# nz0001na/MorphGANformer

Measured on AMD Instinct MI355X. Metric: latent-projection iters/sec @1024^2, k=17 latents, higher is better.
Workload: dtype f32; 1 GPU; configs[1]: single 1024x1024 face per GPU, Wing+LPIPS(squeeze)+MSE literal-mode projection step, noise_mode=random, seeded synthetic weights/targets/landmarks; k=17, z_dim=32, targets_per_gpu=1, parallelism=pair-sharded x1, graph_replay=True, loss_generator_overlap=True, steps_per_forward=32

## Files before the change

### morphganformer_amd/build.py

```python
from __future__ import annotations

import glob
import hashlib
import os
import subprocess
import sys

HERE = os.path.dirname(os.path.abspath(__file__))
ROOT = os.path.dirname(HERE)
CSRC = os.path.join(HERE, "csrc")
OBJ = os.path.join(CSRC, "_obj")
LIB = os.path.join(HERE, "libmgf_hip.so")
SOURCES = ["capi.cpp", "bias_act.hip", "upfirdn2d.hip", "conv_taps.hip", "latent_prep.hip", "attention.hip", "losses.hip", "lpips_stem.hip",
           "embed.hip", "backward.hip", "wino.hip", "wino3.hip", "pointwise.hip", "narrow_conv.hip", "warp.hip", "lbp.hip", "mdf.hip",
           "wino_tconv.hip", "depthwise.hip", "noise_opt.hip"]
HEADERS = [os.path.join(CSRC, "mgf_common.h"), os.path.join(ROOT, "include", "mgf.h")]
HIPCC = os.environ.get("HIPCC", "/opt/rocm/bin/hipcc")
FLAGS = ["--offload-arch=gfx950", "-O3", "-fPIC", "-std=c++17", "-ffp-contract=on", "-Wno-unused-result", "-x", "hip"]
LINK_FLAGS = ["--offload-arch=gfx950", "-shared", "-fPIC"]

_compiler_id = None


def compiler_id() -> str:
    global _compiler_id
    if _compiler_id is None:
        _compiler_id = subprocess.run([HIPCC, "--version"], stdout=subprocess.PIPE, stderr=subprocess.STDOUT, check=True).stdout.decode()
    return _compiler_id


def object_key(src_path: str, flags) -> str:
    h = hashlib.sha256()
    h.update(compiler_id().encode())
    h.update("\0".join(flags).encode())
    for p in [src_path] + HEADERS:
        with open(p, "rb") as f:
            h.update(b"\0" + os.path.basename(p).encode() + b"\0" + f.read())
    return h.hexdigest()[:16]


def _compile_all(obj_dir, flags_for, verbose, force, prune=True):
    os.makedirs(obj_dir, exist_ok=True)
    objs, todo = [], []
    for src in SOURCES:
        sp = os.path.join(CSRC, src)
        flags = flags_for(src)
        op = os.path.join(obj_dir, f"{src}.{object_key(sp, flags)}.o")
        objs.append(op)
        if force or not os.path.exists(op):
            todo.append((src, op, [HIPCC] + flags + ["-c", sp, "-o", op + ".tmp"]))
    procs, finished = [], []

    def start(i):
        src, op, cmd = todo[i]
        if verbose:
            print(" ".join(cmd), flush=True)
        procs.append((src, op, subprocess.Popen(cmd, stdout=subprocess.PIPE, stderr=subprocess.STDOUT)))

    for i in range(min(max_jobs(), len(todo))):
        start(i)
    while len(finished) < len(procs):
        src, op, pr = procs[len(finished)]
        finished.append((src, op, pr, pr.communicate()[0]))
        if len(procs) < len(todo):
            start(len(procs))
    failed = False
    for src, op, pr, out in finished:
        if pr.returncode != 0:
# ... 75 lines not shown
```

### morphganformer_amd/csrc/conv_taps.hip

```cpp
#include "mgf_common.h"
#include <vector>

namespace {

typedef float f32x16 __attribute__((ext_vector_type(16)));
typedef __bf16 bf16x8 __attribute__((ext_vector_type(8)));
typedef unsigned u32x4 __attribute__((ext_vector_type(4)));

constexpr int CK = 8;
constexpr int CKB = 16;
template <int WM, int WN> struct Slots {
    static constexpr int XS = WN == 4 ? 20 : (WN == 3 ? 15 : (WN == 1 ? 19 : 11));
    static constexpr int WS = WM == 2 ? 5 : 3;
};

struct Ones { float v[2048]; constexpr Ones() : v() { for (int i = 0; i < 2048; ++i) v[i] = 1.0f; } };
__device__ const Ones g_ones = Ones();

struct ConvParams {
    float* y;
    const float* x;
    const float* wp;
    const float* in_scale;
    const float* out_scale;
    mgf_conv_desc d;
    mgf_epilogue ep;
    int has_ep;
    int tw, rows;
    int tw_magic;
    int tiles_x, tiles_y;
    int fh, fw;
    int dy_min, dx_min;
    int co_tiles;
    int ksplit;
    int chunks_per_split;
    int off32_ok;
    float* partial;
    int fixed_geo;
    const void* wb;
    int xcd_per;
};

__device__ __forceinline__ float epi(const mgf_epilogue& ep, float v, int n, int co, int oy, int ox, int out_h, int out_w,
                                     int64_t yoff) {
    if (ep.noise) {
        float ns = ep.noise_strength ? *ep.noise_strength : 1.0f;
        int nn = ep.noise_n > 1 ? n : 0;
        v += ep.noise[((int64_t)nn * out_h + oy) * out_w + ox] * ns;
    }
    if (ep.bias) v += ep.bias[co];
    if (ep.act == MGF_ACT_LRELU) v = v > 0.f ? v : v * ep.alpha;
    else if (ep.act == MGF_ACT_RELU) v = v > 0.f ? v : 0.f;
    v *= ep.gain;
    if (ep.residual) v += ep.residual[yoff];
    return v;
}

__host__ __device__ constexpr int tconv_group(int t) { return ((t / 3) == 1 ? 2 : 0) + ((t % 3) == 1 ? 1 : 0); }

struct TileCtx { int n, ks, co0, ty0, tx0, c_begin, c_end; };

template <int WM, int WN, int MODE, bool PIPE, int NTP, int AR = 0>
__global__ __launch_bounds__(256, 2) void conv_taps_kernel(ConvParams p) {
    static_assert(AR == 0 || (PIPE && (NTP == 9 || NTP == 10)), "bf16x3: the pipelined 3x3 / transposed-conv instantiations only");
    constexpr bool FX = NTP == 10 || NTP == 11;
    constexpr int FXW = NTP == 10 ? 33 : 65;
    constexpr int NT = FX ? 9 : NTP;
    constexpr int CO_T = 32 * WM, PX = 128 * WN, NG = MODE == 1 ? 4 : 1;
    constexpr int CKK = AR ? CKB : CK;
    extern __shared__ float lds[];
    const mgf_conv_desc& d = p.d;
    const int T = NT > 0 ? NT : d.ntaps;
    int toffs[MGF_MAX_TAPS];
#pragma unroll
    for (int t = 0; t < MGF_MAX_TAPS; ++t) toffs[t] = t < T ? (d.dy[t] - p.dy_min) * p.fw + (d.dx[t] - p.dx_min) : 0;
    const int chs = p.fh * p.fw;
    const int xs_floats = CKK * chs;
    const int xs_region = AR ? xs_floats : (PIPE ? Slots<WM, WN>::XS * 256 : xs_floats);
    const int buf_floats = AR ? xs_region + 144 * CO_T : (PIPE ? xs_region + Slots<WM, WN>::WS * 1024 : xs_floats + T * CK * CO_T);

    const int tid = threadIdx.x, lane = tid & 63, wave = tid >> 6;
    const int l31 = lane & 31, half = lane >> 5;
    const int l31_ = l31, half_ = half;
    const int TW = p.tw;
    const int rows = p.rows;
    const int ptiles = p.tiles_x * p.tiles_y;
    const int total_items = ptiles * p.co_tiles * d.n * p.ksplit;
    const int plane = d.in_h * d.in_w;
    const int wrow4 = CO_T / 4;
    const int wsz4 = T * CK * wrow4;

    auto decode = [&](int w, TileCtx& c) {
        const int cot = w % p.co_tiles;
        int r = w / p.co_tiles;
        const int pt = r % ptiles;
        r /= ptiles;
        c.ks = r % p.ksplit;
        c.n = r / p.ksplit;
        c.co0 = cot * CO_T;
        c.ty0 = (pt / p.tiles_x) * rows;
        c.tx0 = (pt % p.tiles_x) * TW;
        c.c_begin = c.ks * p.chunks_per_split * CKK;
        c.c_end = c.c_begin + p.chunks_per_split * CKK;
        if (c.c_end > d.cin) c.c_end = d.cin;
        c.n = __builtin_amdgcn_readfirstlane(c.n); c.ks = __builtin_amdgcn_readfirstlane(c.ks); c.co0 = __builtin_amdgcn_readfirstlane(c.co0);
        c.ty0 = __builtin_amdgcn_readfirstlane(c.ty0); c.tx0 = __builtin_amdgcn_readfirstlane(c.tx0);
        c.c_begin = __builtin_amdgcn_readfirstlane(c.c_begin); c.c_end = __builtin_amdgcn_readfirstlane(c.c_end);
    };

    int pbase[WN];
#pragma unroll
    for (int g = 0; g < WN; ++g) {
        const int pix = (wave * WN + g) * 32 + l31;
        const int pr = (pix * p.tw_magic) >> 16, pc = pix - pr * TW;
        pbase[g] = pr < rows ? pr * d.istride * p.fw + pc * d.istride : 0;
    }

    f32x16 acc[NG][WM][WN];
    auto zero_acc = [&]() {
#pragma unroll
        for (int q = 0; q < NG; ++q)
#pragma unroll
            for (int m = 0; m < WM; ++m)
#pragma unroll
                for (int g = 0; g < WN; ++g)
#pragma unroll
                    for (int r = 0; r < 16; ++r) acc[q][m][g][r] = 0.f;
    };
    zero_acc();

    constexpr int XS = Slots<WM, WN>::XS, WS = Slots<WM, WN>::WS;
    unsigned xoff[XS];
    int woff[WS], wch[WS];
    __amdgpu_buffer_rsrc_t rx_l = __builtin_amdgcn_make_buffer_rsrc((void*)p.x, 0, 0, 0x00020000);
    const __amdgpu_buffer_rsrc_t rw_l = __builtin_amdgcn_make_buffer_rsrc((void*)p.wp, 0, -1, 0x00020000);
    __amdgpu_buffer_rsrc_t rs_l = __builtin_amdgcn_make_buffer_rsrc((void*)g_ones.v, 0, -1, 0x00020000);
    const int sc_step = p.in_scale ? 4 : 0;
    auto setup_slots = [&](const TileCtx& c) {
        rx_l = __builtin_amdgcn_make_buffer_rsrc((void*)(p.x + (int64_t)c.n * d.cin * plane), 0, (int)(4u * (unsigned)(d.cin * plane)), 0x00020000);
        if (p.in_scale) rs_l = __builtin_amdgcn_make_buffer_rsrc((void*)(p.in_scale + (int64_t)c.n * d.cin), 0, -1, 0x00020000);
#pragma unroll
        for (int j = 0; j < WS; ++j) {
            int i = tid + 256 * j;
            if (i >= wsz4) i = wsz4 - 1;
            const int c4 = i % wrow4;
            const int rest = i / wrow4;
            wch[j] = rest % CK;
            woff[j] = ((rest / CK) * d.cin + wch[j]) * d.cout_pad + c.co0 + c4 * 4;
        }
        const int iy0 = c.ty0 * d.istride + p.dy_min, ix0 = c.tx0 * d.istride + p.dx_min;
        int ch = tid / chs;
        int r = (tid - ch * chs) / p.fw;
        int q = tid - ch * chs - r * p.fw;
        const int dr = 256 / p.fw, dq = 256 - dr * p.fw;
#pragma unroll
        for (int j = 0; j < XS; ++j) {
            const int i = tid + 256 * j;
            const int iy = iy0 + r, ix = ix0 + q;
            xoff[j] = (i < xs_floats && iy >= 0 && iy < d.in_h && ix >= 0 && ix < d.in_w) ? 4u * (unsigned)(ch * plane + iy * d.in_w + ix) : 0xFFFFFFF0u;
            q += dq; r += dr;
            if (q >= p.fw) { q -= p.fw; ++r; }
            if (r >= p.fh) { r -= p.fh; ++ch; }
            if (r >= p.fh) { r -= p.fh; ++ch; }
        }
    };
    float xr[XS];
    float4 wr[WS];
    float wsc[WS];
    auto load_chunk = [&](int c0) {
        const int xso = (int)(4u * (unsigned)(c0 * plane)), wso = (int)(4u * (unsigned)(c0 * d.cout_pad)), sso = c0 * sc_step;
#pragma unroll
        for (int j = 0; j < XS; ++j) xr[j] = __builtin_bit_cast(float, __builtin_amdgcn_raw_buffer_load_b32(rx_l, xoff[j], xso, 0));
#pragma unroll
        for (int j = 0; j < WS; ++j) {
            wr[j] = __builtin_bit_cast(float4, __builtin_amdgcn_raw_buffer_load_b128(rw_l, 4u * (unsigned)woff[j], wso, 0));
            wsc[j] = __builtin_bit_cast(float, __builtin_amdgcn_raw_buffer_load_b32(rs_l, 4u * (unsigned)wch[j], sso, 0));
        }
    };
    auto store_chunk = [&](float* buf) {
#pragma unroll
        for (int j = 0; j < XS; ++j) buf[tid + 256 * j] = xr[j];
        float* Wd = buf + xs_region;
#pragma unroll
        for (int j = 0; j < WS; ++j) {
            float4 v = wr[j];
            v.x *= wsc[j]; v.y *= wsc[j]; v.z *= wsc[j]; v.w *= wsc[j];
            *reinterpret_cast<float4*>(Wd + (tid + 256 * j) * 4) = v;
        }
    };
    constexpr int XI = AR ? 3 : 1;
    constexpr int WSB = AR ? (36 * CO_T + 255) / 256 : 1;
    const int stid = tid;
    const int h_st = __builtin_amdgcn_readfirstlane(stid >> 7), lp = stid & 127;
    unsigned xoffb[XI];
    unsigned woffb[WSB];
    struct StageSet { float x[XI][8]; u32x4 w[WSB]; float4 s[2]; };
    int itr[XI], itq[XI];
    unsigned wbase0[WSB];
    if (AR) {
#pragma unroll
        for (int j = 0; j < XI; ++j) {
            const int px = lp + 128 * j;
            itr[j] = px / p.fw;
            itq[j] = px - itr[j] * p.fw;
            if (px >= chs) itr[j] = 1 << 20;
        }
#pragma unroll
        for (int j = 0; j < WSB; ++j) {
            int i = stid + 256 * j;
            if (i >= 36 * CO_T) i = 36 * CO_T - 1;
            const int cc = i % CO_T, rest = i / CO_T;
            wbase0[j] = 16u * (unsigned)(rest * d.cout_pad + cc);
        }
    }
    const __amdgpu_buffer_rsrc_t rwb_l = __builtin_amdgcn_make_buffer_rsrc((void*)p.wb, 0, -1, 0x00020000);
    auto setup_slots_b = [&](const TileCtx& c) {
        rx_l = __builtin_amdgcn_make_buffer_rsrc((void*)(p.x + (int64_t)c.n * d.cin * plane), 0, (int)(4u * (unsigned)(d.cin * plane)), 0x00020000);
        if (p.in_scale) rs_l = __builtin_amdgcn_make_buffer_rsrc((void*)(p.in_scale + (int64_t)c.n * d.cin), 0, -1, 0x00020000);
        const int iy0 = c.ty0 * d.istride + p.dy_min, ix0 = c.tx0 * d.istride + p.dx_min;
// ... 133 lines not shown
                            acc[q][m][g] = __builtin_amdgcn_mfma_f32_32x32x2f32(fa[t & 1][kk][m], fb[t & 1][kk][g], acc[q][m][g], 0, 0, 0);
            }
        } else {
            for (int t = 0; t < T; ++t) {
                const int toff = (d.dy[t] - p.dy_min) * p.fw + (d.dx[t] - p.dx_min);
#pragma unroll
                for (int kk = 0; kk < CK / 2; ++kk) {
                    float a[WM], b[WN];
#pragma unroll
                    for (int m = 0; m < WM; ++m) a[m] = Ws[(t * CK + 2 * kk) * CO_T + m * 32];
#pragma unroll
                    for (int g = 0; g < WN; ++g) b[g] = Xs[2 * kk * chs + pbase[g] + toff];
#pragma unroll
                    for (int m = 0; m < WM; ++m)
#pragma unroll
                        for (int g = 0; g < WN; ++g)
                            acc[0][m][g] = __builtin_amdgcn_mfma_f32_32x32x2f32(a[m], b[g], acc[0][m][g], 0, 0, 0);
                }
            }
        }
    };

    const bool partial = p.ksplit > 1;
    const bool do_ep = p.has_ep && !partial;
    const float ep_ns = (do_ep && p.ep.noise) ? (p.ep.noise_strength ? *p.ep.noise_strength : 1.0f) : 0.f;
    auto epilogue = [&](const TileCtx& c) {
        const int n = c.n, co0 = c.co0;
        int half = half_, l31 = l31_;
        asm volatile("" : "+v"(half), "+v"(l31));
        float* yn = partial ? p.partial + ((int64_t)c.ks * d.n + n) * ((int64_t)d.cout * d.out_h * d.y_pitch) : p.y + (int64_t)n * d.y_batch;
        const int64_t y_plane = partial ? (int64_t)d.out_h * d.y_pitch : d.y_plane;
        const int choff = partial ? 0 : d.y_choff;
        const float* osc = (p.out_scale && !partial) ? p.out_scale + (int64_t)n * d.out_scale_stride : nullptr;
        if (MODE == 0 && WM == 1 && d.rgb_out) {
            const int rc = d.rgb_channels;
            const float* wr = d.rgb_w + (int64_t)n * rc * d.cout;
            float wv[4][16], osv[16], bv[16];
#pragma unroll
            for (int r = 0; r < 16; ++r) {
                const int co = (r & 3) + 8 * (r >> 2) + 4 * half;
                const bool ok = co < d.cout;
                osv[r] = (osc && ok) ? osc[co] : 1.0f;
                bv[r] = (do_ep && p.ep.bias && ok) ? p.ep.bias[co] : 0.f;
#pragma unroll
                for (int cc = 0; cc < 4; ++cc) wv[cc][r] = (cc < rc && ok) ? wr[cc * d.cout + co] : 0.f;
            }
#pragma unroll
            for (int g = 0; g < WN; ++g) {
                const int pix = (wave * WN + g) * 32 + l31;
                const int pr = (pix * p.tw_magic) >> 16;
                const int ty = c.ty0 + pr, tx = c.tx0 + (pix - pr * TW);
                const int oy = ty * d.ostride + d.oy[0], ox = tx * d.ostride + d.ox[0];
                const bool ovalid = pr < rows && ty < d.tile_h && tx < d.tile_w && oy < d.out_h && ox < d.out_w;
                float nz = 0.f;
                if (do_ep && p.ep.noise && ovalid) nz = p.ep.noise[((int64_t)(p.ep.noise_n > 1 ? n : 0) * d.out_h + oy) * d.out_w + ox] * ep_ns;
                float sum[4] = {0.f, 0.f, 0.f, 0.f};
#pragma unroll
                for (int r = 0; r < 16; ++r) {
                    float v = acc[0][0][g][r] * osv[r];
                    if (do_ep) {
                        v += nz;
                        v += bv[r];
                        if (p.ep.act == MGF_ACT_LRELU) v = v > 0.f ? v : v * p.ep.alpha;
                        else if (p.ep.act == MGF_ACT_RELU) v = v > 0.f ? v : 0.f;
                        v *= p.ep.gain;
                    }
// ... 225 lines not shown
                        mfma_chunk_b(curb);
                        if (more) store_chunk_b(S0, nxtb);
                    } else {
                        if (more) load_chunk(cur.c_begin + (c + 1) * CK);
                        mfma_chunk(curb);
                        if (more) store_chunk(nxtb);
                    }
                    __syncthreads();
                    b ^= 1;
                }
                epilogue(cur);
                zero_acc();
                slot += slot_step;
                if (slot >= slot_end) break;
                decode(wbase + slot, cur);
            }
        }
    } else {
        const int w = p.xcd_per > 0 ? (int)(blockIdx.x & 7) * p.xcd_per + (int)(blockIdx.x >> 3) : (int)blockIdx.x;
        if (w >= total_items || (p.xcd_per > 0 && (int)(blockIdx.x >> 3) >= p.xcd_per)) return;
        TileCtx cur;
        decode(w, cur);
        const int nchunks = (cur.c_end - cur.c_begin + CK - 1) / CK;
        for (int c = 0; c < nchunks; ++c) {
            __syncthreads();
            stage_direct(cur, cur.c_begin + c * CK, lds);
            __syncthreads();
            mfma_chunk(lds);
        }
        epilogue(cur);
    }
}

__global__ __launch_bounds__(256) void splitk_reduce_kernel(ConvParams p) {
    const mgf_conv_desc& d = p.d;
    const int64_t per_n = (int64_t)d.cout * d.out_h * d.out_w;
    const int64_t total = per_n * d.n;
    const int64_t pplane = (int64_t)d.out_h * d.y_pitch;
    const int64_t slice = (int64_t)d.n * d.cout * pplane;
    for (int64_t i = (int64_t)blockIdx.x * 256 + threadIdx.x; i < total; i += (int64_t)gridDim.x * 256) {
        const int ox = (int)(i % d.out_w);
        int64_t r = i / d.out_w;
        const int oy = (int)(r % d.out_h); r /= d.out_h;
        const int co = (int)(r % d.cout);
        const int n = (int)(r / d.cout);
        const int64_t poff = ((int64_t)n * d.cout + co) * pplane + (int64_t)oy * d.y_pitch + ox;
        float v = 0.f;
        const float* pp = p.partial + poff;
        int s = 0;
        for (; s + 8 <= p.ksplit; s += 8) {
            float a[8];
#pragma unroll
            for (int u = 0; u < 8; ++u) a[u] = pp[(int64_t)(s + u) * slice];
#pragma unroll
            for (int u = 0; u < 8; ++u) v += a[u];
        }
        for (; s + 4 <= p.ksplit; s += 4) {
            const float a0 = pp[(int64_t)s * slice], a1 = pp[(int64_t)(s + 1) * slice];
            const float a2 = pp[(int64_t)(s + 2) * slice], a3 = pp[(int64_t)(s + 3) * slice];
            v += a0; v += a1; v += a2; v += a3;
        }
        for (; s < p.ksplit; ++s) v += pp[(int64_t)s * slice];
        if (p.out_scale) v *= p.out_scale[(int64_t)n * d.out_scale_stride + co];
        const int64_t yoff = (int64_t)n * d.y_batch + (int64_t)(d.y_choff + co) * d.y_plane + (int64_t)oy * d.y_pitch + ox;
        if (p.has_ep) v = epi(p.ep, v, n, co, oy, ox, d.out_h, d.out_w, yoff);
        p.y[yoff] = v;
    }
}

struct ProfRec { hipEvent_t e0, e1; int wm, wn, mode, pipe, nt, ksplit; double flops, bytes; const char* name; };
bool g_prof_on = false;
std::vector<ProfRec> g_prof;

struct ProfScope {
    hipStream_t st; bool on;
    ProfScope(hipStream_t s, int wm, int wn, int mode, int pipe, int nt, const ConvParams& p) : st(s), on(g_prof_on) {
        if (!on) return;
        ProfRec r;
        r.name = nullptr;
        r.wm = wm; r.wn = wn; r.mode = mode; r.pipe = pipe; r.nt = nt; r.ksplit = p.ksplit;
        const mgf_conv_desc& d = p.d;
        r.flops = mode == 1 ? 2.0 * 9 * d.cin * (double)d.cout * d.in_h * d.in_w * d.n
                            : 2.0 * d.ntaps * d.cin * (double)d.cout * d.tile_h * d.tile_w * d.n;
        r.bytes = 4.0 * ((double)d.n * d.cin * d.in_h * d.in_w + (double)d.ntaps * d.cin * d.cout +
                         (double)d.n * (d.rgb_out ? d.rgb_channels : d.cout) * d.out_h * d.out_w);
        (void)hipEventCreate(&r.e0); (void)hipEventCreate(&r.e1);
        (void)hipEventRecord(r.e0, st);
        g_prof.push_back(r);
    }
    ~ProfScope() { if (on) (void)hipEventRecord(g_prof.back().e1, st); }
};

template <int MODE>
int launch_conv_bf(const ConvParams& p_in, hipStream_t st) {
    ConvParams p = p_in;
    constexpr int WM = 1, WN = 2, CO_T = 32;
    const int chs = p.fh * p.fw;
    const size_t lds = 2 * ((size_t)16 * chs + (size_t)144 * CO_T) * sizeof(float);
    if (2 * chs > 768 || p.d.cin % CKB != 0 || lds > 80 * 1024) {
        mgf_set_error("conv_taps(bf16x3): footprint %d x %d / %d input channels not supported", p.fh, p.fw, p.d.cin);
        return MGF_EUNSUPPORTED;
    }
    const int64_t items = (int64_t)p.tiles_x * p.tiles_y * p.co_tiles * p.d.n * p.ksplit;
    const int64_t resident = (int64_t)MGF_NUM_CU * 2;
    dim3 grid((unsigned)(items < resident ? items : resident));
    p.xcd_per = 0;
    if (items >= 16) {
        p.xcd_per = (int)((items + 7) / 8);
        if (grid.x % 8 != 0) grid.x = (grid.x + 7) / 8 * 8;
    }
    auto kern1 = conv_taps_kernel<WM, WN, MODE, true, (MODE == 1 ? 10 : 9), 1>;
    static bool attr_set = false;
    if (!attr_set) {
        hipError_t e = hipFuncSetAttribute((const void*)kern1, hipFuncAttributeMaxDynamicSharedMemorySize, 80 * 1024);
        if (e != hipSuccess) { mgf_set_error("conv_taps(bf16x3): cannot raise dynamic LDS: %s", hipGetErrorString(e)); return MGF_ELAUNCH; }
        attr_set = true;
    }
    {
        ProfScope ps(st, WM, WN, MODE, 1, MODE == 1 ? 10 : 9, p);
        if (ps.on) g_prof.back().name = MODE == 1 ? "conv_taps_kernel<1, 2, 1, true, 10, 1>" : "conv_taps_kernel<1, 2, 0, true, 9, 1>";
        hipLaunchKernelGGL(kern1, grid, dim3(256), lds, st, p);
    }
    if (p.ksplit > 1) {
        const int64_t total = (int64_t)p.d.n * p.d.cout * p.d.out_h * p.d.out_w;
        hipLaunchKernelGGL(splitk_reduce_kernel, dim3(mgf_stream_grid(total, 256, 2)), dim3(256), 0, st, p);
    }
    return MGF_OK;
}

template <int WM, int WN, int MODE>
int launch_conv(const ConvParams& p_in, hipStream_t st) {
    ConvParams p = p_in;
    constexpr int CO_T = 32 * WM;
    const size_t buf = ((size_t)CK * p.fh * p.fw + (size_t)p.d.ntaps * CK * CO_T) * sizeof(float);
    const bool pipe = (size_t)CK * p.fh * p.fw <= (size_t)Slots<WM, WN>::XS * 256 &&
                      (size_t)p.d.ntaps * CK * CO_T / 4 <= (size_t)Slots<WM, WN>::WS * 256 &&
                      256 / p.fw + 2 <= 2 * p.fh &&
                      p.d.cin % CK == 0;
    const size_t lds = pipe ? 2 * ((size_t)Slots<WM, WN>::XS * 256 + (size_t)Slots<WM, WN>::WS * 1024) * sizeof(float) : buf;
    if (lds > 160 * 1024) { mgf_set_error("conv_taps: tile needs %zu bytes of LDS (> 160 KiB)", lds); return MGF_EUNSUPPORTED; }
    const int64_t items = (int64_t)p.tiles_x * p.tiles_y * p.co_tiles * p.d.n * p.ksplit;
    static const char* res_env = mgf_knob("MGF_RESIDENT");
    const int64_t resident = (int64_t)MGF_NUM_CU * (res_env ? atoi(res_env) : ((WM == 1 && WN == 2 && MODE == 0) ? 3 : 2));
    dim3 grid((unsigned)(pipe && (p.d.ntaps == 9 || ((p.d.ntaps == 1 || p.d.ntaps == 7 || p.d.ntaps == 3) && MODE == 0)) ? (items < resident ? items : resident) : items));
    static const char* xcd_env = mgf_knob("MGF_XCD");
    p.xcd_per = 0;
    if (!(xcd_env && xcd_env[0] == '0') && items >= 16) {
        p.xcd_per = (int)((items + 7) / 8);
        if (grid.x % 8 != 0) grid.x = (grid.x + 7) / 8 * 8;
    }
    const int nt = p.d.ntaps;
    if (pipe && nt == 9 && MODE == 1 && WN == 2 && p.fixed_geo) {
        ProfScope ps(st, WM, WN, MODE, 1, 10, p);
        hipLaunchKernelGGL((conv_taps_kernel<WM, (MODE == 1 ? 2 : WN), MODE, true, (MODE == 1 ? 10 : 9)>), grid, dim3(256), lds, st, p);
    } else if (pipe && nt == 9 && MODE == 0 && WN == 1 && p.fixed_geo == 2) {
        ProfScope ps(st, WM, WN, MODE, 1, 11, p);
        hipLaunchKernelGGL((conv_taps_kernel<WM, (MODE == 0 ? 1 : WN), MODE, true, (MODE == 0 ? 11 : 9)>), grid, dim3(256), lds, st, p);
    } else if (pipe && nt == 9) {
        ProfScope ps(st, WM, WN, MODE, 1, 9, p);
        hipLaunchKernelGGL((conv_taps_kernel<WM, WN, MODE, true, 9>), grid, dim3(256), lds, st, p);
    } else if (pipe && (nt == 7 || nt == 3) && MODE == 0) {
        ProfScope ps(st, WM, WN, MODE, 1, nt, p);
        if (nt == 7) hipLaunchKernelGGL((conv_taps_kernel<WM, WN, MODE == 1 ? 0 : MODE, true, 7>), grid, dim3(256), lds, st, p);
        else hipLaunchKernelGGL((conv_taps_kernel<WM, WN, MODE == 1 ? 0 : MODE, true, 3>), grid, dim3(256), lds, st, p);
    } else if (pipe && nt == 1 && MODE == 0) {
        ProfScope ps(st, WM, WN, MODE, 1, 1, p);
        hipLaunchKernelGGL((conv_taps_kernel<WM, WN, MODE == 1 ? 0 : MODE, true, 1>), grid, dim3(256), lds, st, p);
    } else {
        ProfScope ps(st, WM, WN, MODE, 0, nt == 9 ? 9 : 0, p);
        auto kern9 = conv_taps_kernel<WM, WN, MODE, false, 9>;
        auto kern0 = conv_taps_kernel<WM, WN, MODE == 1 ? 0 : MODE, false, 0>;
        const size_t lds1 = buf;
        const void* fn = (nt == 9) ? (const void*)kern9 : (const void*)kern0;
        if (lds1 > 64 * 1024) {
            hipError_t e = hipFuncSetAttribute(fn, hipFuncAttributeMaxDynamicSharedMemorySize, (int)lds1);
            if (e != hipSuccess) { mgf_set_error("conv_taps: cannot raise dynamic LDS to %zu: %s", lds1, hipGetErrorString(e)); return MGF_ELAUNCH; }
        }
        if (nt == 9) hipLaunchKernelGGL(kern9, grid, dim3(256), lds1, st, p);
        else hipLaunchKernelGGL(kern0, grid, dim3(256), lds1, st, p);
    }
    if (p.ksplit > 1) {
        const int64_t total = (int64_t)p.d.n * p.d.cout * p.d.out_h * p.d.out_w;
        hipLaunchKernelGGL(splitk_reduce_kernel, dim3(mgf_stream_grid(total, 256, 2)), dim3(256), 0, st, p);
    }
    return MGF_OK;
// ... 8 lines not shown
        const int64_t r = i / cout_pad;
        const int ci = (int)(r % cin);
        const int t = (int)(r / cin);
        float v = 0.f;
        if (co < cout) {
            int ky = t / kw, kx = t % kw;
            if (flip) { ky = kh - 1 - ky; kx = kw - 1 - kx; }
            v = w[(((int64_t)co * cin + ci) * kh + ky) * kw + kx] * gain;
        }
        wp[i] = v;
    }
    if (wsq) {
        const int64_t tot2 = (int64_t)cout * cin;
        for (int64_t i = (int64_t)blockIdx.x * blockDim.x + threadIdx.x; i < tot2; i += (int64_t)gridDim.x * blockDim.x) {
            float s = 0.f;
            for (int t = 0; t < T; ++t) { float v = w[i * T + t] * gain; s += v * v; }
            wsq[i] = s;
        }
    }
}

}

extern "C" int mgf_conv_profile_begin(void) {
    for (auto& r : g_prof) { (void)hipEventDestroy(r.e0); (void)hipEventDestroy(r.e1); }
    g_prof.clear();
    g_prof_on = true;
    return MGF_OK;
}

void mgf_prof_external_begin(hipStream_t st, const char* name, double flops, double bytes) {
    if (!g_prof_on) return;
    ProfRec r;
    r.name = name; r.wm = r.wn = r.mode = r.pipe = r.nt = 0; r.ksplit = 1; r.flops = flops; r.bytes = bytes;
    (void)hipEventCreate(&r.e0); (void)hipEventCreate(&r.e1);
    (void)hipEventRecord(r.e0, st);
    g_prof.push_back(r);
}
void mgf_prof_external_end(hipStream_t st) {
    if (g_prof_on && !g_prof.empty()) (void)hipEventRecord(g_prof.back().e1, st);
}

extern "C" int mgf_conv_profile_end(mgf_conv_prof_rec* out, int32_t max_recs) {
    g_prof_on = false;
    int n = 0;
    for (auto& r : g_prof) {
        if (hipEventSynchronize(r.e1) != hipSuccess) { mgf_set_error("conv_profile_end: event sync failed"); return MGF_ELAUNCH; }
        float ms = 0.f;
        (void)hipEventElapsedTime(&ms, r.e0, r.e1);
        if (out && n < max_recs) {
            mgf_conv_prof_rec& o = out[n];
            if (r.name) snprintf(o.kernel, sizeof(o.kernel), "%s", r.name);
            else snprintf(o.kernel, sizeof(o.kernel), "conv_taps_kernel<%d, %d, %d, %s, %d, 0>", r.wm, r.wn, r.mode, r.pipe ? "true" : "false", r.nt);
            o.flops = r.flops; o.bytes = r.bytes; o.seconds = ms * 1e-3; o.ksplit = r.ksplit;
        }
        ++n;
        (void)hipEventDestroy(r.e0); (void)hipEventDestroy(r.e1);
    }
    g_prof.clear();
    return n;
}

constexpr int TB_POS = 64, TB_CK = 32, TB_LINE = TB_POS / 2 + 1, TB_LP = TB_LINE + 1;
__global__ __launch_bounds__(256) void tconv_border_kernel(float* t, const float* x, const float* wp, const float* in_scale,
                                                           const float* out_scale, int cin, int h, int w, int cout, int cout_pad,
                                                           int64_t pitch, int64_t plane, int64_t batch, int64_t os_stride, int col_groups) {
    __shared__ float Ws[3][TB_CK][64];
    __shared__ float Xl[TB_CK][TB_LP];
    const int tid = threadIdx.x, n = blockIdx.z, co0 = blockIdx.y * 64;
    const int lane = tid & 63, l31 = lane & 31, half = lane >> 5, wv = __builtin_amdgcn_readfirstlane(tid >> 6);
    const bool col = (int)blockIdx.x < col_groups;
    const int p0 = (col ? blockIdx.x : blockIdx.x - col_groups) * TB_POS;
    const int npos = col ? 2 * h + 1 : 2 * w;
    const int lim = col ? h : w;
    const int tap0 = col ? 2 : 6, tapstep = col ? 3 : 1;
    const float* xn = x + (int64_t)n * cin * h * w;
    const int64_t hw = (int64_t)h * w;
    constexpr int XR = (TB_CK * TB_LINE + 255) / 256, WR = 3 * TB_CK * 64 / 256;
    int xsrc[XR];
#pragma unroll
    for (int r = 0; r < XR; ++r) {
        const int e = tid + 256 * r, jj = e % TB_LINE;
        const int i = p0 / 2 - 1 + jj;
        xsrc[r] = (e < TB_CK * TB_LINE && i >= 0 && i < lim) ? (col ? i * w + (w - 1) : (h - 1) * w + i) : -1;
    }
// ... 110 lines not shown
                        MGF_EUNSUPPORTED, "conv_taps: epilogue activation %d unsupported", ep->act);
    ConvParams p;
    p.y = y; p.x = x; p.wp = wp; p.wb = wb; p.in_scale = in_scale; p.out_scale = out_scale; p.d = d;
    p.has_ep = ep != nullptr;
    if (ep) { p.ep = *ep; if (p.ep.act == 0) p.ep.act = MGF_ACT_LINEAR; } else { p.ep = mgf_epilogue{}; p.ep.gain = 1.f; }
    int dy_min = d.dy[0], dy_max = d.dy[0], dx_min = d.dx[0], dx_max = d.dx[0];
    for (int t = 1; t < d.ntaps; ++t) {
        dy_min = d.dy[t] < dy_min ? d.dy[t] : dy_min; dy_max = d.dy[t] > dy_max ? d.dy[t] : dy_max;
        dx_min = d.dx[t] < dx_min ? d.dx[t] : dx_min; dx_max = d.dx[t] > dx_max ? d.dx[t] : dx_max;
    }
    p.dy_min = dy_min; p.dx_min = dx_min;
    int mode = 0;
    if (d.ngroups == 4) {
        MGF_REQUIRE(d.ntaps == 9 && d.ostride == 2 && d.istride == 1, MGF_EUNSUPPORTED, "conv_taps: 4-group mode is the 3x3 stride-2 transposed conv");
        for (int t = 0; t < 9; ++t) {
            MGF_REQUIRE(d.group[t] == tconv_group(t), MGF_EINVAL, "conv_taps: tap %d must belong to parity group %d", t, tconv_group(t));
        }
        MGF_REQUIRE(ep == nullptr, MGF_EUNSUPPORTED, "conv_taps: the transposed-conv mode has no fused epilogue (it feeds the FIR pass)");
        MGF_REQUIRE(d.y_pitch % 2 == 0 && d.y_plane % 2 == 0 && d.y_batch % 2 == 0 && ((uintptr_t)y % 8) == 0, MGF_EINVAL,
                    "conv_taps: transposed-conv output needs even pitch/plane/batch strides and 8-byte alignment");
        mode = 1;
    }
    int tw_log2 = 5;
    while (tw_log2 > 2 && (1 << (tw_log2 - 1)) >= d.tile_w) --tw_log2;
    int TW = 1 << tw_log2;
    int wm = 1, wn = 2;
    static const char* small_env = mgf_knob("MGF_SMALL_TILES");
    const bool small = (int64_t)d.tile_h * d.tile_w <= 128 && !(small_env && small_env[0] == '0');
    if (wb) {
        MGF_REQUIRE(d.ntaps == 9 && d.istride == 1 && !small && TW == 32 && d.cin % CKB == 0, MGF_EUNSUPPORTED,
                    "conv_taps(bf16x3): needs 9 taps, stride 1, a map of more than 128 positions at least 32 wide and cin %% 16 == 0");
    }
    if (mode == 1 && small) wn = 1;
    if (mode == 0 && wb) { wm = 1; wn = 2; }
    else if (mode == 0) {
        if (d.cout_pad % 64 == 0 && d.cout > 32) { wm = 2; wn = small ? 1 : 2; }
        else if (small) { wm = 1; wn = 1; }
        else if ((int64_t)d.tile_h * d.tile_w >= 512 * 64) { wm = 1; wn = d.ntaps == 9 ? 3 : 4; }
        static const char* s2_env = mgf_knob("MGF_S2_SMALL");
        if (d.istride == 2 && !(s2_env && s2_env[0] == '0')) wn = 1;
        static const char* force = mgf_knob("MGF_CONV_TILE");
        if (force && force[0] && force[1] == ',' && force[2]) {
            const int fm = force[0] - '0', fn = force[2] - '0';
            if ((fm == 2 && fn == 2 && d.cout_pad % 64 == 0) || (fm == 1 && (fn == 2 || fn == 3 || fn == 4))) { wm = fm; wn = fn; }
        }
    }
    const int PX = 128 * wn;
    int rows = PX / TW;
    if (mode == 1) {
        static const char* tw_env = mgf_knob("MGF_TCONV_TW");
        int64_t best = mgf_cdiv(d.tile_w, TW) * mgf_cdiv(d.tile_h, rows) * 9;
        for (int tw = 8; tw <= 64 && !(tw_env && tw_env[0] == '0') && !wb; ++tw) {
            const int r = PX / tw;
            const int fh_ = r + (dy_max - dy_min), fw_ = tw + (dx_max - dx_min);
            if (256 / fw_ + 2 > 2 * fh_ || (size_t)CK * fh_ * fw_ > (size_t)(wn == 1 ? Slots<1, 1>::XS : Slots<1, 2>::XS) * 256) continue;
            const int64_t tiles = mgf_cdiv(d.tile_w, tw) * mgf_cdiv(d.tile_h, r);
            if (tiles * 10 < best) { best = tiles * 10; TW = tw; rows = r; }
        }
    }
    if (mode == 0 && !wb && d.istride == 1 && TW == 32 && d.tile_w > 16) {
        const size_t cap = (size_t)(wn == 4 ? Slots<1, 4>::XS : (wn == 3 ? Slots<1, 3>::XS : (wn == 1 ? Slots<1, 1>::XS : Slots<1, 2>::XS))) * 256;
        auto fits = [&](int tw) {
            const int r = PX / tw, fh_ = r + (dy_max - dy_min), fw_ = tw + (dx_max - dx_min);
            return (size_t)CK * fh_ * fw_ <= cap && 256 / fw_ + 2 <= 2 * fh_;
        };
        if (!fits(32) && fits(16)) { TW = 16; rows = PX / 16; }
    }
    p.tw = TW; p.rows = rows; p.tw_magic = (65536 + TW - 1) / TW;
    p.tiles_x = (int)mgf_cdiv(d.tile_w, TW);
    p.tiles_y = (int)mgf_cdiv(d.tile_h, rows);
    p.fh = (rows - 1) * d.istride + (dy_max - dy_min) + 1;
    p.fw = (TW - 1) * d.istride + (dx_max - dx_min) + 1;
    p.fixed_geo = 0;
    if (mode == 1 && p.fh == 9 && p.fw == 33) {
        p.fixed_geo = 1;
        for (int t = 0; t < 9; ++t)
            if (d.dy[t] != ((t / 3) == 2 ? -1 : 0) || d.dx[t] != ((t % 3) == 2 ? -1 : 0)) p.fixed_geo = 0;
        static const char* fg_env = mgf_knob("MGF_TCONV_FIXED");
        if (fg_env && fg_env[0] == '0') p.fixed_geo = 0;
    }
    if (mode == 0 && d.ntaps == 9 && d.istride == 2 && p.fh == 9 && p.fw == 65) {
        p.fixed_geo = 2;
        for (int t = 0; t < 9; ++t)
            if (d.dy[t] - dy_min != t / 3 || d.dx[t] - dx_min != t % 3) p.fixed_geo = 0;
        static const char* fg_env = mgf_knob("MGF_TCONV_FIXED");
        if (fg_env && fg_env[0] == '0') p.fixed_geo = 0;
    }
    p.co_tiles = d.cout_pad / (32 * wm);
    const int64_t base_wgs = (int64_t)p.tiles_x * p.tiles_y * p.co_tiles * d.n;
    const int nchunks = (int)mgf_cdiv(d.cin, wb ? CKB : CK);
    int ksplit = 1;
    static const int splitk_below = [] { const char* e = mgf_knob("MGF_SPLITK_BELOW"); return e ? atoi(e) : 256; }();
    if (d.workspace && base_wgs < splitk_below && nchunks >= 4 && !d.rgb_out) {
        static const int splitk_target = [] { const char* e = mgf_knob("MGF_SPLITK_TARGET"); return e ? atoi(e) : 1024; }();
        ksplit = (int)mgf_cdiv(splitk_target, base_wgs);
        if (ksplit > nchunks / 2) ksplit = nchunks / 2;
        const int64_t slice = (int64_t)d.n * d.cout * d.out_h * d.y_pitch;
        while (ksplit > 1 && slice * ksplit > d.workspace_floats) --ksplit;
        if (ksplit < 1) ksplit = 1;
    }
    p.chunks_per_split = (int)mgf_cdiv(nchunks, ksplit);
    ksplit = (int)mgf_cdiv(nchunks, p.chunks_per_split);
    p.ksplit = ksplit;
    p.partial = d.workspace;
    p.off32_ok = ((int64_t)(d.y_choff + d.cout_pad) * d.y_plane < (1LL << 30)) && ((int64_t)d.cout_pad * d.out_h * d.y_pitch < (1LL << 30));
    MGF_REQUIRE((int64_t)p.tiles_x * p.tiles_y * p.co_tiles * d.n * ksplit <= INT32_MAX, MGF_ETOOBIG, "conv_taps: grid too large");
    hipStream_t st = (hipStream_t)stream;
    int rc;
    if (wb) {
        MGF_REQUIRE(mode == 0 || p.fixed_geo == 1, MGF_EUNSUPPORTED, "conv_taps(bf16x3): the transposed conv needs its canonical tile (9 x 33 footprint)");
        rc = mode == 1 ? launch_conv_bf<1>(p, st) : launch_conv_bf<0>(p, st);
    }
    else if (mode == 1) rc = wn == 1 ? launch_conv<1, 1, 1>(p, st) : launch_conv<1, 2, 1>(p, st);
    else if (wn == 1) rc = wm == 2 ? launch_conv<2, 1, 0>(p, st) : launch_conv<1, 1, 0>(p, st);
    else if (wm == 2) rc = launch_conv<2, 2, 0>(p, st);
    else if (wn == 4) rc = launch_conv<1, 4, 0>(p, st);
    else if (wn == 3) rc = launch_conv<1, 3, 0>(p, st);
    else rc = launch_conv<1, 2, 0>(p, st);
    if (rc != MGF_OK) return rc;
    MGF_CHECK_LAUNCH("conv_taps");
    return MGF_OK;
}

extern "C" int mgf_conv_taps_f32(float* y, const float* x, const float* wp, const float* in_scale, const float* out_scale,
                                 const mgf_conv_desc* dd, const mgf_epilogue* ep, mgf_stream_t stream) {
    MGF_REQUIRE(wp, MGF_EINVAL, "conv_taps: null pointer");
    return conv_taps_dispatch(y, x, wp, nullptr, in_scale, out_scale, dd, ep, stream);
}

extern "C" int mgf_conv_taps_bf16x3_f32(float* y, const float* x, const void* wb, const float* in_scale, const float* out_scale,
                                        const mgf_conv_desc* dd, const mgf_epilogue* ep, mgf_stream_t stream) {
    MGF_REQUIRE(wb && ((uintptr_t)wb % 16) == 0, MGF_EINVAL, "conv_taps(bf16x3): the split weights must be 16-byte aligned");
    return conv_taps_dispatch(y, x, nullptr, wb, in_scale, out_scale, dd, ep, stream);
}
```

Measured before the change: 781.2 iters/s.

## Pack several small-map batch samples into one conv_taps tile

For small spatial maps (early generator layers at 4x4/8x8 with k=17 latents), the 3x3 conv kernel now packs several batch samples into a single pixel tile. Previously each sample occupied a tile that was mostly idle lanes. A new packed kernel instantiation maps lanes to (sample,row,col), applies per-sample input scales on the activation side, and has its own epilogue for both normal and transposed convs. This is meant to cut wasted MFMA lanes and workgroup count on small layers. In exchange it adds more per-element scale loads, a simplified epilogue path, and changes to the split-k and wm heuristics.

After: 781.8 iters/s, median of 2. Within noise of the previous version (+0.1%).

```diff
diff --git a/morphganformer_amd/build.py b/morphganformer_amd/build.py
--- a/morphganformer_amd/build.py
+++ b/morphganformer_amd/build.py
@@ -15,6 +15,7 @@
            "embed.hip", "backward.hip", "wino.hip", "wino3.hip", "pointwise.hip", "narrow_conv.hip", "warp.hip", "lbp.hip", "mdf.hip",
            "wino_tconv.hip", "depthwise.hip", "noise_opt.hip"]
 HEADERS = [os.path.join(CSRC, "mgf_common.h"), os.path.join(ROOT, "include", "mgf.h")]
+OWN_HEADERS = {"conv_taps.hip": [os.path.join(CSRC, "conv_pack_map.h")]}
 HIPCC = os.environ.get("HIPCC", "/opt/rocm/bin/hipcc")
 FLAGS = ["--offload-arch=gfx950", "-O3", "-fPIC", "-std=c++17", "-ffp-contract=on", "-Wno-unused-result", "-x", "hip"]
 LINK_FLAGS = ["--offload-arch=gfx950", "-shared", "-fPIC"]
@@ -33,7 +34,7 @@
     h = hashlib.sha256()
     h.update(compiler_id().encode())
     h.update("\0".join(flags).encode())
-    for p in [src_path] + HEADERS:
+    for p in [src_path] + HEADERS + OWN_HEADERS.get(os.path.basename(src_path), []):
         with open(p, "rb") as f:
             h.update(b"\0" + os.path.basename(p).encode() + b"\0" + f.read())
     return h.hexdigest()[:16]
diff --git a/morphganformer_amd/csrc/conv_pack_map.h b/morphganformer_amd/csrc/conv_pack_map.h
--- /dev/null
+++ b/morphganformer_amd/csrc/conv_pack_map.h
@@ -0,0 +1,46 @@
+#pragma once
+#ifndef __HIPCC__
+#define MGF_PACK_HD
+#else
+#define MGF_PACK_HD __host__ __device__
+#endif
+
+struct PackGeo {
+    int S;
+    int R, tw;
+    int bh, fw;
+    int tw_magic;
+    int r_magic;
+    int bh_magic;
+};
+
+struct PackLane { int s, r, c, lds; };
+
+MGF_PACK_HD inline PackLane pack_lane(const PackGeo& g, int pix) {
+    PackLane l;
+    const int vr = (pix * g.tw_magic) >> 16;
+    l.c = pix - vr * g.tw;
+    l.s = (vr * g.r_magic) >> 16;
+    l.r = vr - l.s * g.R;
+    l.lds = l.s < g.S ? (l.s * g.bh + l.r) * g.fw + l.c : 0;
+    return l;
+}
+
+MGF_PACK_HD inline long pack_x_offset(const PackGeo& g, int ch, int vrow, int q, int dy_min, int dx_min, int cin, int in_h, int in_w,
+                                      int nvalid, int* sample) {
+    const int s = (vrow * g.bh_magic) >> 16;
+    const int iy = vrow - s * g.bh + dy_min, ix = q + dx_min;
+    *sample = s;
+    if (s >= nvalid || iy < 0 || iy >= in_h || ix < 0 || ix >= in_w) return -1;
+    return ((long)(s * cin + ch) * in_h + iy) * in_w + ix;
+}
+
+MGF_PACK_HD inline long pack_store_offset(const PackLane& l, const PackGeo& g, int transposed, int a, int out_h, int out_w, long pitch,
+                                          int* pair) {
+    *pair = 0;
+    if (l.s >= g.S) return -1;
+    const int oy = transposed ? 2 * l.r + a : l.r, ox = transposed ? 2 * l.c : l.c;
+    if (oy >= out_h || ox >= out_w) return -1;
+    *pair = transposed && ox + 1 < out_w;
+    return (long)oy * pitch + ox;
+}
diff --git a/morphganformer_amd/csrc/conv_taps.hip b/morphganformer_amd/csrc/conv_taps.hip
--- a/morphganformer_amd/csrc/conv_taps.hip
+++ b/morphganformer_amd/csrc/conv_taps.hip
@@ -1,4 +1,5 @@
 #include "mgf_common.h"
+#include "conv_pack_map.h"
 #include <vector>
 
 namespace {
@@ -39,6 +40,8 @@
     int fixed_geo;
     const void* wb;
     int xcd_per;
+    PackGeo pk;
+    int n_items;
 };
 
 __device__ __forceinline__ float epi(const mgf_epilogue& ep, float v, int n, int co, int oy, int ox, int out_h, int out_w,
@@ -60,8 +63,9 @@
 
 struct TileCtx { int n, ks, co0, ty0, tx0, c_begin, c_end; };
 
-template <int WM, int WN, int MODE, bool PIPE, int NTP, int AR = 0>
-__global__ __launch_bounds__(256, 2) void conv_taps_kernel(ConvParams p) {
+template <int WM, int WN, int MODE, bool PIPE, int NTP, int AR, bool PK>
+__device__ __forceinline__ void conv_taps_body(const ConvParams& p) {
+    static_assert(!PK || (PIPE && NTP == 9 && AR == 0), "packed tiles: the pipelined 3x3 / transposed-conv f32 instantiations only");
     static_assert(AR == 0 || (PIPE && (NTP == 9 || NTP == 10)), "bf16x3: the pipelined 3x3 / transposed-conv instantiations only");
     constexpr bool FX = NTP == 10 || NTP == 11;
     constexpr int FXW = NTP == 10 ? 33 : 65;
@@ -85,7 +89,8 @@
     const int TW = p.tw;
     const int rows = p.rows;
     const int ptiles = p.tiles_x * p.tiles_y;
-    const int total_items = ptiles * p.co_tiles * d.n * p.ksplit;
+    const int total_items = ptiles * p.co_tiles * p.n_items * p.ksplit;
+    const int PS = PK ? p.pk.S : 0;
     const int plane = d.in_h * d.in_w;
     const int wrow4 = CO_T / 4;
     const int wsz4 = T * CK * wrow4;
@@ -97,6 +102,7 @@
         r /= ptiles;
         c.ks = r % p.ksplit;
         c.n = r / p.ksplit;
+        if (PK) c.n *= PS;
         c.co0 = cot * CO_T;
         c.ty0 = (pt / p.tiles_x) * rows;
         c.tx0 = (pt % p.tiles_x) * TW;
@@ -114,6 +120,7 @@
         const int pix = (wave * WN + g) * 32 + l31;
         const int pr = (pix * p.tw_magic) >> 16, pc = pix - pr * TW;
         pbase[g] = pr < rows ? pr * d.istride * p.fw + pc * d.istride : 0;
+        if (PK) pbase[g] = pack_lane(p.pk, pix).lds;
     }
 
     f32x16 acc[NG][WM][WN];
@@ -131,6 +138,7 @@
 
     constexpr int XS = Slots<WM, WN>::XS, WS = Slots<WM, WN>::WS;
     unsigned xoff[XS];
+    unsigned soff[XS];
     int woff[WS], wch[WS];
     __amdgpu_buffer_rsrc_t rx_l = __builtin_amdgcn_make_buffer_rsrc((void*)p.x, 0, 0, 0x00020000);
     const __amdgpu_buffer_rsrc_t rw_l = __builtin_amdgcn_make_buffer_rsrc((void*)p.wp, 0, -1, 0x00020000);
@@ -139,6 +147,12 @@
     auto setup_slots = [&](const TileCtx& c) {
         rx_l = __builtin_amdgcn_make_buffer_rsrc((void*)(p.x + (int64_t)c.n * d.cin * plane), 0, (int)(4u * (unsigned)(d.cin * plane)), 0x00020000);
         if (p.in_scale) rs_l = __builtin_amdgcn_make_buffer_rsrc((void*)(p.in_scale + (int64_t)c.n * d.cin), 0, -1, 0x00020000);
+        const int nvalid = d.n - c.n < PS ? d.n - c.n : PS;
+        if (PK) {
+            rx_l = __builtin_amdgcn_make_buffer_rsrc((void*)(p.x + (int64_t)c.n * d.cin * plane), 0, (int)(4u * (unsigned)(nvalid * d.cin * plane)), 0x00020000);
+            if (p.in_scale) rs_l = __builtin_amdgcn_make_buffer_rsrc((void*)(p.in_scale + (int64_t)c.n * d.cin), 0, (int)(4u * (unsigned)(nvalid * d.cin)), 0x00020000);
+            else rs_l = __builtin_amdgcn_make_buffer_rsrc((void*)g_ones.v, 0, 4 * 2048, 0x00020000);
+        }
 #pragma unroll
         for (int j = 0; j < WS; ++j) {
             int i = tid + 256 * j;
@@ -158,6 +172,12 @@
             const int i = tid + 256 * j;
             const int iy = iy0 + r, ix = ix0 + q;
             xoff[j] = (i < xs_floats && iy >= 0 && iy < d.in_h && ix >= 0 && ix < d.in_w) ? 4u * (unsigned)(ch * plane + iy * d.in_w + ix) : 0xFFFFFFF0u;
+            if (PK) {
+                int sm;
+                const long xo = i < xs_floats ? pack_x_offset(p.pk, ch, r, q, p.dy_min, p.dx_min, d.cin, d.in_h, d.in_w, nvalid, &sm) : -1;
+                xoff[j] = xo >= 0 ? 4u * (unsigned)xo : 0xFFFFFFF0u;
+                soff[j] = xo >= 0 ? 4u * (unsigned)((p.in_scale ? sm * d.cin : 0) + ch) : 0xFFFFFFF0u;
+            }
             q += dq; r += dr;
             if (q >= p.fw) { q -= p.fw; ++r; }
             if (r >= p.fh) { r -= p.fh; ++ch; }
@@ -167,6 +187,7 @@
     float xr[XS];
     float4 wr[WS];
     float wsc[WS];
+    float xsv[XS];
     auto load_chunk = [&](int c0) {
         const int xso = (int)(4u * (unsigned)(c0 * plane)), wso = (int)(4u * (unsigned)(c0 * d.cout_pad)), sso = c0 * sc_step;
 #pragma unroll
@@ -174,17 +195,21 @@
 #pragma unroll
         for (int j = 0; j < WS; ++j) {
             wr[j] = __builtin_bit_cast(float4, __builtin_amdgcn_raw_buffer_load_b128(rw_l, 4u * (unsigned)woff[j], wso, 0));
-            wsc[j] = __builtin_bit_cast(float, __builtin_amdgcn_raw_buffer_load_b32(rs_l, 4u * (unsigned)wch[j], sso, 0));
+            if (!PK) wsc[j] = __builtin_bit_cast(float, __builtin_amdgcn_raw_buffer_load_b32(rs_l, 4u * (unsigned)wch[j], sso, 0));
+        }
+        if (PK) {
+#pragma unroll
+            for (int j = 0; j < XS; ++j) xsv[j] = __builtin_bit_cast(float, __builtin_amdgcn_raw_buffer_load_b32(rs_l, soff[j], sso, 0));
         }
     };
     auto store_chunk = [&](float* buf) {
 #pragma unroll
-        for (int j = 0; j < XS; ++j) buf[tid + 256 * j] = xr[j];
+        for (int j = 0; j < XS; ++j) buf[tid + 256 * j] = PK ? xr[j] * xsv[j] : xr[j];
         float* Wd = buf + xs_region;
 #pragma unroll
         for (int j = 0; j < WS; ++j) {
             float4 v = wr[j];
-            v.x *= wsc[j]; v.y *= wsc[j]; v.z *= wsc[j]; v.w *= wsc[j];
+            if (!PK) { v.x *= wsc[j]; v.y *= wsc[j]; v.z *= wsc[j]; v.w *= wsc[j]; }
             *reinterpret_cast<float4*>(Wd + (tid + 256 * j) * 4) = v;
         }
     };
@@ -384,6 +409,56 @@
         const int64_t y_plane = partial ? (int64_t)d.out_h * d.y_pitch : d.y_plane;
         const int choff = partial ? 0 : d.y_choff;
         const float* osc = (p.out_scale && !partial) ? p.out_scale + (int64_t)n * d.out_scale_stride : nullptr;
+        if (PK) {
+#pragma unroll
+            for (int g = 0; g < WN; ++g) {
+                const PackLane pl = pack_lane(p.pk, (wave * WN + g) * 32 + l31);
+                const int ln = n + pl.s;
+                if (pl.s >= PS || ln >= d.n) continue;
+                float* yl = partial ? p.partial + ((int64_t)c.ks * d.n + ln) * ((int64_t)d.cout * d.out_h * d.y_pitch) : p.y + (int64_t)ln * d.y_batch;
+                const float* osl = osc ? osc + (int64_t)pl.s * d.out_scale_stride : nullptr;
+                int pair0, pair1;
+                const int64_t off0 = pack_store_offset(pl, p.pk, MODE == 1, 0, d.out_h, d.out_w, d.y_pitch, &pair0);
+                const int64_t off1 = MODE == 1 ? pack_store_offset(pl, p.pk, 1, 1, d.out_h, d.out_w, d.y_pitch, &pair1) : -1;
+                float nz = 0.f;
+                if (MODE == 0 && do_ep && p.ep.noise && off0 >= 0)
+                    nz = p.ep.noise[((int64_t)(p.ep.noise_n > 1 ? ln : 0) * d.out_h + pl.r) * d.out_w + pl.c] * ep_ns;
+#pragma unroll
+                for (int m = 0; m < WM; ++m) {
+#pragma unroll
+                    for (int r = 0; r < 16; ++r) {
+                        const int co = co0 + m * 32 + (r & 3) + 8 * (r >> 2) + 4 * half;
+                        if (co >= d.cout) continue;
+                        const float os = osl ? osl[co] : 1.0f;
+                        float* yc = yl + (int64_t)(choff + co) * y_plane;
+                        if (MODE == 0) {
+                            if (off0 < 0) continue;
+                            float v = acc[0][m][g][r] * os;
+                            if (do_ep) {
+                                v += nz;
+                                if (p.ep.bias) v += p.ep.bias[co];
+                                if (p.ep.act == MGF_ACT_LRELU) v = v > 0.f ? v : v * p.ep.alpha;
+                                else if (p.ep.act == MGF_ACT_RELU) v = v > 0.f ? v : 0.f;
+                                const float rv = p.ep.residual ? p.ep.residual[(int64_t)ln * d.y_batch + (int64_t)(choff + co) * y_plane + off0] : 0.f;
+                                v = v * p.ep.gain + rv;
+                            }
+                            yc[off0] = v;
+                        } else {
+#pragma unroll
+                            for (int a2 = 0; a2 < 2; ++a2) {
+                                const int64_t off = a2 ? off1 : off0;
+                                if (off < 0) continue;
+                                const float v0 = acc[NG == 4 ? 2 * a2 : 0][m][g][r] * os;
+                                const float v1 = acc[NG == 4 ? 2 * a2 + 1 : 0][m][g][r] * os;
+                                if (a2 ? pair1 : pair0) *reinterpret_cast<float2*>(yc + off) = make_float2(v0, v1);
+                                else yc[off] = v0;
+                            }
+                        }
+                    }
+                }
+            }
+            return;
+        }
         if (MODE == 0 && WM == 1 && d.rgb_out) {
             const int rc = d.rgb_channels;
             const float* wr = d.rgb_w + (int64_t)n * rc * d.cout;
@@ -675,6 +750,12 @@
     }
 }
 
+template <int WM, int WN, int MODE, bool PIPE, int NTP, int AR = 0>
+__global__ __launch_bounds__(256, 2) void conv_taps_kernel(ConvParams p) { conv_taps_body<WM, WN, MODE, PIPE, NTP, AR, false>(p); }
+
+template <int WM, int WN, int MODE>
+__global__ __launch_bounds__(256, 2) void conv_taps_packed_kernel(ConvParams p) { conv_taps_body<WM, WN, MODE, true, 9, 0, true>(p); }
+
 __global__ __launch_bounds__(256) void splitk_reduce_kernel(ConvParams p) {
     const mgf_conv_desc& d = p.d;
     const int64_t per_n = (int64_t)d.cout * d.out_h * d.out_w;
@@ -711,7 +792,7 @@
     }
 }
 
-struct ProfRec { hipEvent_t e0, e1; int wm, wn, mode, pipe, nt, ksplit; double flops, bytes; const char* name; };
+struct ProfRec { hipEvent_t e0, e1; int wm, wn, mode, pipe, nt, ksplit, packed; double flops, bytes; const char* name; };
 bool g_prof_on = false;
 std::vector<ProfRec> g_prof;
 
@@ -721,7 +802,7 @@
         if (!on) return;
         ProfRec r;
         r.name = nullptr;
-        r.wm = wm; r.wn = wn; r.mode = mode; r.pipe = pipe; r.nt = nt; r.ksplit = p.ksplit;
+        r.wm = wm; r.wn = wn; r.mode = mode; r.pipe = pipe; r.nt = nt; r.ksplit = p.ksplit; r.packed = p.pk.S > 0;
         const mgf_conv_desc& d = p.d;
         r.flops = mode == 1 ? 2.0 * 9 * d.cin * (double)d.cout * d.in_h * d.in_w * d.n
                             : 2.0 * d.ntaps * d.cin * (double)d.cout * d.tile_h * d.tile_w * d.n;
@@ -744,7 +825,7 @@
         mgf_set_error("conv_taps(bf16x3): footprint %d x %d / %d input channels not supported", p.fh, p.fw, p.d.cin);
         return MGF_EUNSUPPORTED;
     }
-    const int64_t items = (int64_t)p.tiles_x * p.tiles_y * p.co_tiles * p.d.n * p.ksplit;
+    const int64_t items = (int64_t)p.tiles_x * p.tiles_y * p.co_tiles * p.n_items * p.ksplit;
     const int64_t resident = (int64_t)MGF_NUM_CU * 2;
     dim3 grid((unsigned)(items < resident ? items : resident));
     p.xcd_per = 0;
@@ -782,7 +863,8 @@
                       p.d.cin % CK == 0;
     const size_t lds = pipe ? 2 * ((size_t)Slots<WM, WN>::XS * 256 + (size_t)Slots<WM, WN>::WS * 1024) * sizeof(float) : buf;
     if (lds > 160 * 1024) { mgf_set_error("conv_taps: tile needs %zu bytes of LDS (> 160 KiB)", lds); return MGF_EUNSUPPORTED; }
-    const int64_t items = (int64_t)p.tiles_x * p.tiles_y * p.co_tiles * p.d.n * p.ksplit;
+    if (p.pk.S && !(pipe && p.d.ntaps == 9)) { mgf_set_error("conv_taps: a packed tile needs the pipelined 3x3 kernel"); return MGF_EUNSUPPORTED; }
+    const int64_t items = (int64_t)p.tiles_x * p.tiles_y * p.co_tiles * p.n_items * p.ksplit;
     static const char* res_env = mgf_knob("MGF_RESIDENT");
     const int64_t resident = (int64_t)MGF_NUM_CU * (res_env ? atoi(res_env) : ((WM == 1 && WN == 2 && MODE == 0) ? 3 : 2));
     dim3 grid((unsigned)(pipe && (p.d.ntaps == 9 || ((p.d.ntaps == 1 || p.d.ntaps == 7 || p.d.ntaps == 3) && MODE == 0)) ? (items < resident ? items : resident) : items));
@@ -793,7 +875,16 @@
         if (grid.x % 8 != 0) grid.x = (grid.x + 7) / 8 * 8;
     }
     const int nt = p.d.ntaps;
-    if (pipe && nt == 9 && MODE == 1 && WN == 2 && p.fixed_geo) {
+    if (p.pk.S) {
+        ProfScope ps(st, WM, WN, MODE, 1, 9, p);
+#ifdef MGF_TUNING_HOOKS
+        constexpr bool inst = WN == 1 || (WN == 2 && WM == 1 && MODE == 1);
+#else
+        constexpr bool inst = WN == 1;
+#endif
+        if (inst) hipLaunchKernelGGL((conv_taps_packed_kernel<(inst ? WM : 1), (inst ? WN : 1), MODE>), grid, dim3(256), lds, st, p);
+        else { mgf_set_error("conv_taps: no packed kernel for a %d x %d tile", WM, WN); return MGF_EUNSUPPORTED; }
+    } else if (pipe && nt == 9 && MODE == 1 && WN == 2 && p.fixed_geo) {
         ProfScope ps(st, WM, WN, MODE, 1, 10, p);
         hipLaunchKernelGGL((conv_taps_kernel<WM, (MODE == 1 ? 2 : WN), MODE, true, (MODE == 1 ? 10 : 9)>), grid, dim3(256), lds, st, p);
     } else if (pipe && nt == 9 && MODE == 0 && WN == 1 && p.fixed_geo == 2) {
@@ -868,7 +959,7 @@
 void mgf_prof_external_begin(hipStream_t st, const char* name, double flops, double bytes) {
     if (!g_prof_on) return;
     ProfRec r;
-    r.name = name; r.wm = r.wn = r.mode = r.pipe = r.nt = 0; r.ksplit = 1; r.flops = flops; r.bytes = bytes;
+    r.name = name; r.wm = r.wn = r.mode = r.pipe = r.nt = r.packed = 0; r.ksplit = 1; r.flops = flops; r.bytes = bytes;
     (void)hipEventCreate(&r.e0); (void)hipEventCreate(&r.e1);
     (void)hipEventRecord(r.e0, st);
     g_prof.push_back(r);
@@ -887,6 +978,7 @@
         if (out && n < max_recs) {
             mgf_conv_prof_rec& o = out[n];
             if (r.name) snprintf(o.kernel, sizeof(o.kernel), "%s", r.name);
+            else if (r.packed) snprintf(o.kernel, sizeof(o.kernel), "conv_taps_packed_kernel<%d, %d, %d>", r.wm, r.wn, r.mode);
             else snprintf(o.kernel, sizeof(o.kernel), "conv_taps_kernel<%d, %d, %d, %s, %d, 0>", r.wm, r.wn, r.mode, r.pipe ? "true" : "false", r.nt);
             o.flops = r.flops; o.bytes = r.bytes; o.seconds = ms * 1e-3; o.ksplit = r.ksplit;
         }
@@ -1063,6 +1155,11 @@
                     "conv_taps(bf16x3): needs 9 taps, stride 1, a map of more than 128 positions at least 32 wide and cin %% 16 == 0");
     }
     if (mode == 1 && small) wn = 1;
+    static const char* pack_env = mgf_knob("MGF_SMALL_PACK");
+    const int pack_knob = pack_env ? atoi(pack_env) : 1;
+    const bool can_pack = small && pack_knob != 0 && d.n > 1 && !wb && !d.rgb_out && d.ntaps == 9 && d.istride == 1 && d.cin % CK == 0 &&
+                          d.tile_w <= 64 && (mode == 1 || (d.ostride == 1 && d.oy[0] == 0 && d.ox[0] == 0));
+    int pack_s = 0;
     if (mode == 0 && wb) { wm = 1; wn = 2; }
     else if (mode == 0) {
         if (d.cout_pad % 64 == 0 && d.cout > 32) { wm = 2; wn = small ? 1 : 2; }
@@ -1076,9 +1173,24 @@
             if ((fm == 2 && fn == 2 && d.cout_pad % 64 == 0) || (fm == 1 && (fn == 2 || fn == 3 || fn == 4))) { wm = fm; wn = fn; }
         }
     }
+    static const int splitk_below = [] { const char* e = mgf_knob("MGF_SPLITK_BELOW"); return e ? atoi(e) : 256; }();
+    if (can_pack && wn <= 2) {
+        const int bh = d.tile_h + (dy_max - dy_min), fw = d.tile_w + (dx_max - dx_min);
+        auto fit = [&](int wn_) {
+            const int xs = wn_ == 1 ? (wm == 2 ? Slots<2, 1>::XS : Slots<1, 1>::XS) : (wm == 2 ? Slots<2, 2>::XS : Slots<1, 2>::XS);
+            int s_ = (int)(128 * wn_ / ((int64_t)d.tile_h * d.tile_w));
+            while (s_ > 1 && (size_t)CK * s_ * bh * fw > (size_t)xs * 256) --s_;
+            return s_;
+        };
+        pack_s = fit(wn);
+        if (mode == 1 && wn == 1 && pack_knob == 2 && fit(2) > 2 * fit(1)) { wn = 2; pack_s = fit(2); }
+        if (pack_s < 2 || 256 / fw + 2 > 2 * pack_s * bh) pack_s = 0;
+        if (pack_s && mode == 0 && wm == 2 && pack_knob != 3 && 2 * (d.cout_pad / 64) * mgf_cdiv(d.n, pack_s) < splitk_below) wm = 1;
+    }
     const int PX = 128 * wn;
     int rows = PX / TW;
-    if (mode == 1) {
+    if (pack_s) { TW = d.tile_w; rows = pack_s * d.tile_h; }
+    if (mode == 1 && !pack_s) {
         static const char* tw_env = mgf_knob("MGF_TCONV_TW");
         int64_t best = mgf_cdiv(d.tile_w, TW) * mgf_cdiv(d.tile_h, rows) * 9;
         for (int tw = 8; tw <= 64 && !(tw_env && tw_env[0] == '0') && !wb; ++tw) {
@@ -1102,6 +1214,16 @@
     p.tiles_y = (int)mgf_cdiv(d.tile_h, rows);
     p.fh = (rows - 1) * d.istride + (dy_max - dy_min) + 1;
     p.fw = (TW - 1) * d.istride + (dx_max - dx_min) + 1;
+    p.pk = PackGeo{};
+    p.n_items = d.n;
+    if (pack_s) {
+        PackGeo& g = p.pk;
+        g.S = pack_s; g.R = d.tile_h; g.tw = TW; g.bh = d.tile_h + (dy_max - dy_min); g.fw = p.fw;
+        g.tw_magic = p.tw_magic; g.r_magic = (65536 + g.R - 1) / g.R; g.bh_magic = (65536 + g.bh - 1) / g.bh;
+        p.tiles_y = 1;
+        p.fh = pack_s * g.bh;
+        p.n_items = (int)mgf_cdiv(d.n, pack_s);
+    }
     p.fixed_geo = 0;
     if (mode == 1 && p.fh == 9 && p.fw == 33) {
         p.fixed_geo = 1;
@@ -1118,10 +1240,9 @@
         if (fg_env && fg_env[0] == '0') p.fixed_geo = 0;
     }
     p.co_tiles = d.cout_pad / (32 * wm);
-    const int64_t base_wgs = (int64_t)p.tiles_x * p.tiles_y * p.co_tiles * d.n;
+    const int64_t base_wgs = (int64_t)p.tiles_x * p.tiles_y * p.co_tiles * p.n_items;
     const int nchunks = (int)mgf_cdiv(d.cin, wb ? CKB : CK);
     int ksplit = 1;
-    static const int splitk_below = [] { const char* e = mgf_knob("MGF_SPLITK_BELOW"); return e ? atoi(e) : 256; }();
     if (d.workspace && base_wgs < splitk_below && nchunks >= 4 && !d.rgb_out) {
         static const int splitk_target = [] { const char* e = mgf_knob("MGF_SPLITK_TARGET"); return e ? atoi(e) : 1024; }();
         ksplit = (int)mgf_cdiv(splitk_target, base_wgs);
@@ -1135,7 +1256,7 @@
     p.ksplit = ksplit;
     p.partial = d.workspace;
     p.off32_ok = ((int64_t)(d.y_choff + d.cout_pad) * d.y_plane < (1LL << 30)) && ((int64_t)d.cout_pad * d.out_h * d.y_pitch < (1LL << 30));
-    MGF_REQUIRE((int64_t)p.tiles_x * p.tiles_y * p.co_tiles * d.n * ksplit <= INT32_MAX, MGF_ETOOBIG, "conv_taps: grid too large");
+    MGF_REQUIRE((int64_t)p.tiles_x * p.tiles_y * p.co_tiles * p.n_items * ksplit <= INT32_MAX, MGF_ETOOBIG, "conv_taps: grid too large");
     hipStream_t st = (hipStream_t)stream;
     int rc;
     if (wb) {
```
